# haoosz/FFR-Net

Hardware: AMD Instinct MI355X
Metric: face embeddings/sec (IR-SE50 + RecNet forward, 112x112 fp32) at batch 256 per GPU (higher is better)
Workload: dtype f32; 1 GPU; configs[2]: IR-SE50 + RecBlock (spatial+channel) forward, batch 256 per GPU, 112x112x3 fp32 -> f_new,f [512]; + all-gather of embeddings and pair cosine scores (112x96 of the BASELINE label cannot be embedded by the reference: BASELINE.md); batch_per_gpu=256, global_batch=256, parallelism=image-sharded x1, RCCL all-gather of embeddings

## Files before the change

ffr-net_amd/csrc/conv.cpp:

```cpp
#include "engine_internal.h"

namespace ffr_eng {

#ifdef FFR_TRACE
static int trace_igemm(ffr_handle* h, IgemmArgs& a, int tile, int nblocks, long long units, hipStream_t st) {
    unsigned long long* dbuf = nullptr;
    HIPCK(h, hipMalloc((void**)&dbuf, (size_t)nblocks * 8 * sizeof(unsigned long long)));
    a.trace = dbuf;
    HIPCK(h, launch_igemm(a, tile, nblocks, st));
    HIPCK(h, hipStreamSynchronize(st));
    std::vector<unsigned long long> t((size_t)nblocks * 8);
    HIPCK(h, hipMemcpy(t.data(), dbuf, t.size() * 8, hipMemcpyDeviceToHost));
    HIPCK(h, hipFree(dbuf));
    a.trace = nullptr;
    double acc[4] = {0, 0, 0, 0}, segs = 0, e1 = 0, e2 = 0, ghz = 0;
    unsigned long long r0 = ~0ull, r1 = 0, smax = 0;
    for (int b = 0; b < nblocks; ++b) {
        const unsigned long long* q = &t[(size_t)b * 8];
        for (int k = 0; k < 4; ++k) acc[k] += (double)q[k];
        segs += (double)q[4];
        ghz += (double)(q[0] + q[1] + q[2] + q[3]) / ((double)(q[6] - q[5]) * 10.0);
        e1 += (double)(q[7] >> 32); e2 += (double)(q[7] & 0xffffffffull);
        if (q[5] < r0) r0 = q[5];
        if (q[5] > smax) smax = q[5];
        if (q[6] > r1) r1 = q[6];
    }
    fprintf(stderr, "[igemm trace] tile %d blocks %d units %lld nkt %d segs/blk %.2f | per segment: setup %.0f prologue %.0f "
                    "loop %.0f (%.0f per K-tile) epilogue %.0f (first barrier at %.0f, C in LDS at %.0f) cyc | span %.1f us, starts within %.1f us, shader clock %.2f GHz\n",
            tile, nblocks, units, a.nkt, segs / nblocks, acc[0] / segs, acc[1] / segs, acc[2] / segs,
            acc[2] / ((double)units), acc[3] / segs, e1 / segs, e2 / segs, (double)(r1 - r0) / 100.0, (double)(smax - r0) / 100.0, ghz / nblocks);
    return FFR_OK;
}

static int trace_wino_mixed(ffr_handle* h, WinoMixedArgs& f, const ConvW& L, const ConvCall& c, hipStream_t st) {
    const int nbm = wino_mixed_blocks_launched(c.N, c.H, c.W, L.cout_pad, f.xcd_pairs);
    unsigned long long* dbuf = nullptr;
    HIPCK(h, hipMalloc((void**)&dbuf, (size_t)nbm * 12 * sizeof(unsigned long long)));
    HIPCK(h, hipMemsetAsync(dbuf, 0, (size_t)nbm * 12 * sizeof(unsigned long long), st));
    f.trace = dbuf;
    hipEvent_t e0, e1;
    HIPCK(h, hipEventCreate(&e0)); HIPCK(h, hipEventCreate(&e1));
    HIPCK(h, hipEventRecord(e0, st));
    HIPCK(h, launch_wino_fused_mixed(f, st));
    HIPCK(h, hipEventRecord(e1, st));
    HIPCK(h, hipStreamSynchronize(st));
    float ev_ms = 0.f;
    HIPCK(h, hipEventElapsedTime(&ev_ms, e0, e1));
    hipEventDestroy(e0); hipEventDestroy(e1);
    std::vector<unsigned long long> tr((size_t)nbm * 12);
    HIPCK(h, hipMemcpy(tr.data(), dbuf, tr.size() * 8, hipMemcpyDeviceToHost));
    HIPCK(h, hipFree(dbuf));
    double pro[4] = {0, 0, 0, 0}, loop[4] = {0, 0, 0, 0}, ep1[4] = {0, 0, 0, 0}, ep2[4] = {0, 0, 0, 0}, clk[4] = {0, 0, 0, 0};
    int cnt[4] = {0, 0, 0, 0};
// ... 240 lines not shown
        c2.x = c.x + px * c.in_pitch;
        c2.out = c.out + px * c.out_pitch;
        if (c.resid) c2.resid = c.resid + px * c.res_pitch;
        if (c.tile_sums) c2.tile_sums = c.tile_sums + (size_t)p.n_main * ((c.H + 3) / 4) * ((c.W + 3) / 4) * L.cout_pad;
        if (p.side) {
            HIPCK(h, hipEventRecord(h->ev_fork, st));
            HIPCK(h, hipStreamWaitEvent(p.side, h->ev_fork, 0));
            RC(run_conv(h, L, c2, p.side));
            HIPCK(h, hipEventRecord(h->ev_join, p.side));
            RC(run_conv(h, L, c1, st));
            HIPCK(h, hipStreamWaitEvent(st, h->ev_join, 0));
            return FFR_OK;
        }
        RC(run_conv(h, L, c1, st));
        return run_conv(h, L, c2, st);
    }
    IgemmArgs a{};
    a.x = c.x; a.w = L.w; a.bias = L.bias; a.slope = L.slope; a.resid = c.resid; a.out = c.out; a.zero = h->zero;
    a.N = c.N; a.H = c.H; a.W = c.W; a.Ho = Ho; a.Wo = Wo;
    a.in_pitch = c.in_pitch; a.cin_pad = L.cin_pad; a.R = L.R; a.S = L.S; a.stride = L.stride; a.pad = L.pad; a.pad_mode = L.pad_mode;
    a.M = (int)M; a.KK = L.R * L.S * L.cin_pad; a.nkt = a.KK / 32; a.nbatch = 1;
    a.cout_pad = L.cout_pad; a.cout_store = c.cout_store; a.out_pitch = c.out_pitch; a.out_coff = c.out_coff;
    a.res_pitch = c.res_pitch; a.border_bias = L.border; a.flags = c.flags;
    if (L.w3 && h->opt.igemm_split) { a.w3 = L.w3; a.w3_pstride = (long long)L.cout_pad * a.KK; }
    return run_gemm(h, a, c, flops, bytes, st);
}

int gemm_rows(ffr_handle* h, const Work& w, const float* A, int a_pitch, int K_pad, const float* W, const float* bias,
              int N_pad, float* out, int out_pitch, long long rows, const float* resid, int res_pitch, int flags,
              hipStream_t st) {
    ConvW cw;
    cw.cin = K_pad; cw.cin_pad = K_pad; cw.cout = N_pad; cw.cout_pad = N_pad; cw.R = 1; cw.S = 1; cw.stride = 1; cw.pad = 0;
    cw.pad_mode = 0; cw.border = 0; cw.w = const_cast<float*>(W); cw.bias = bias ? const_cast<float*>(bias) : h->zero;
    cw.slope = nullptr; cw.wu = nullptr;
    ConvCall c = conv_call(w, ConvForce::Direct);
    c.x = A; c.N = 1; c.H = 1; c.W = (int)rows; c.in_pitch = a_pitch; c.resid = resid; c.res_pitch = res_pitch;
    c.out = out; c.out_pitch = out_pitch; c.out_coff = 0; c.cout_store = N_pad; c.flags = flags;
    return run_conv(h, cw, c, st);
}

int gemm_batched(ffr_handle* h, const Work& w, const float* A, long long a_bstride, int K_pad, const float* W,
                 long long w_bstride, int N_pad, float* out, int out_pitch, long long out_bstride, int M, int nbatch,
                 hipStream_t st) {
    const double fl = 2.0 * nbatch * (double)M * N_pad * K_pad;
    return igemm_batched(h, conv_call(w, ConvForce::Direct), A, a_bstride, K_pad, W, w_bstride, N_pad, out, out_pitch, out_bstride, M,
                         nbatch, fl, 4.0 * nbatch * ((double)M * K_pad + (double)N_pad * K_pad + (double)M * N_pad), fl, st);
}
// ... 3 lines not shown
```

ffr-net_amd/csrc/engine.cpp:

```cpp
#include "engine_internal.h"

using namespace ffr;
using namespace ffr_eng;

namespace ffr_eng {

std::string g_err = "";

int fail(ffr_handle* h, int code, const char* fmt, ...) {
    char buf[512];
    va_list ap;
    va_start(ap, fmt);
    vsnprintf(buf, sizeof buf, fmt, ap);
    va_end(ap);
    if (h) h->err = buf; else g_err = buf;
    return code;
}

struct PlanLayer { ConvW* L; std::string name; int net; };

std::vector<PlanLayer> plan_layers(const ffr_handle* hc) {
    ffr_handle* h = const_cast<ffr_handle*>(hc);
    std::vector<PlanLayer> v;
    if (h->enc_loaded)
// ... 483 lines not shown
        RC(forward()); RC(compare(0));
        RC(read());
        if (err(0) <= half || p == 0) break;
    }
    if (achieved) for (int t = 0; t < 4; ++t) achieved[t] = have[t] ? rel(0, t) : -1.0;
    sv.keep = true;
    bool changed = false;
    for (auto& pr : sv.plan) changed |= pr.first->direct != pr.second;
    if (changed) plan_changed(h);
    else h->mixed_ready_n = 0;
    return FFR_OK;
}

namespace {
struct OptEntry { const char* name; int ffr_eng::Options::*i; long long ffr_eng::Options::*l; long long lo, hi; };
const OptEntry OPTIONS[] = {
    {"wino", &Options::wino, nullptr, 0, 1}, {"wino_mincin", &Options::wino_mincin, nullptr, 0, 1 << 20},
    {"wino_fused", &Options::wino_fused, nullptr, 0, 1},
    {"wf_phased_maxk", &Options::wf_phased_maxk, nullptr, 0, 1 << 20}, {"wf_minblocks", nullptr, &Options::wf_minblocks, 0, 1LL << 40},
    {"se_maxtiles", &Options::se_maxtiles, nullptr, 0, 1 << 20}, {"wf_tailsplit", &Options::wf_tailsplit, nullptr, 0, 1},
    {"gemm_stream", &Options::gemm_stream, nullptr, 0, 1}, {"sk_minunits", &Options::sk_minunits, nullptr, 1, 1 << 20},
    {"combine_v", &Options::combine_v, nullptr, 0, 1}, {"wf_mixed", &Options::wf_mixed, nullptr, 0, 1},
    {"channel_rows", &Options::channel_rows, nullptr, 0, 4}, {"igemm_split", &Options::igemm_split, nullptr, 0, 1},
    {"wf_trace", &Options::wf_trace, nullptr, 0, 1}, {"igemm_trace", &Options::igemm_trace, nullptr, 0, 1},
};
const OptEntry* find_option(const char* name) {
    if (name) for (const OptEntry& e : OPTIONS) if (!strcmp(e.name, name)) return &e;
    return nullptr;
}
}

int ffr_set_option(ffr_handle* h, const char* name, long long value) {
    if (!h) return fail(nullptr, FFR_ERR_ARG, "null handle");
    const OptEntry* e = find_option(name);
    if (!e) return fail(h, FFR_ERR_ARG, "ffr_set_option: unknown option '%s'", name ? name : "(null)");
    if (value < e->lo || value > e->hi) return fail(h, FFR_ERR_ARG, "ffr_set_option: %s = %lld is outside [%lld, %lld]", name, value, e->lo, e->hi);
    if (e->i == &Options::channel_rows && value == 3) return fail(h, FFR_ERR_ARG, "ffr_set_option: channel_rows is 0 (auto), 1, 2 or 4");
#ifndef FFR_TRACE
    if ((e->i == &Options::wf_trace || e->i == &Options::igemm_trace) && value)
        return fail(h, FFR_ERR_UNSUPPORTED, "ffr_set_option: %s needs a -DFFR_TRACE build of the library (tools/trace_build.py)", name);
#endif
    const long long old = e->i ? (long long)(h->opt.*(e->i)) : h->opt.*(e->l);
    if (old != value) ++h->generation;
    if (e->i) h->opt.*(e->i) = (int)value; else h->opt.*(e->l) = value;
    return FFR_OK;
}
// ... 154 lines not shown
```

ffr-net_amd/csrc/engine_internal.h:

```cpp
#pragma once
#include <hip/hip_runtime.h>

#include <algorithm>
#include <chrono>
#include <cmath>
#include <cstdarg>
#include <cstdio>
#include <cstdlib>
#include <cstring>
#include <initializer_list>
#include <map>
#include <string>
#include <vector>

#include "../../include/ffrnet.h"
#include "../../include/ffrnet_train.h"
#include "ffr_kernels.h"

namespace ffr_eng {

using namespace ffr;

struct TrainState;

// ... 12 lines not shown
};

struct Block {
    int cin = 0, depth = 0, stride = 1;
    bool has_sc = false;
    ConvW c1, c2, sc;
    float* fc1 = nullptr;
    float* fc2 = nullptr;
};

struct Options {
    int wino = 1;
    int wino_mincin = 64;
    int wino_fused = 1;
    int wf_phased_maxk = 128;
    long long wf_minblocks = 200;
    int se_maxtiles = 256;
    int wf_tailsplit = 1;
    int gemm_stream = 1;
    int sk_minunits = 18;
    int wf_mixed = 1;
    int channel_rows = 0;
    int igemm_split = 1;
    int combine_v = 1;
    int wf_trace = 0, igemm_trace = 0;
};

struct ProfRec {
    hipEvent_t e0, e1;
    int kc;
    double flops, bytes, fexec, fuse;
    bool side;
};

}

struct ffr_handle {
    int device = 0;
    int num_cus = 256;
    hipStream_t side = nullptr;
    hipEvent_t ev_fork = nullptr, ev_join = nullptr;
    std::string err;
    float* zero = nullptr;
    std::vector<void*> enc_allocs, rec_allocs;
    bool enc_loaded = false, rec_loaded = false;
    size_t enc_weight_bytes = 0, rec_weight_bytes = 0;
// ... 197 lines not shown
```

ffr-net_amd/csrc/ffr_kernels.h:

```cpp
#pragma once
#include <hip/hip_runtime.h>
#include <stdint.h>

#ifdef FFR_TRACE
#define FFR_TRACE_ON(p) ((p) != nullptr)
#else
#define FFR_TRACE_ON(p) false
#endif

namespace ffr {

struct IgemmArgs {
    const float* x;
    const float* w;
    const float* bias;
    const float* slope;
    const float* resid;
    float* out;
    const float* zero;
    float* partial;
    int* tickets;
    unsigned long long* trace;
    int N, H, W, Ho, Wo, in_pitch, cin_pad, R, S, stride, pad, pad_mode;
    int M, KK, nkt, granule;
    int nbatch;
    long long x_bstride, w_bstride, out_bstride;
    int cout_pad, cout_store, out_pitch, out_coff, res_pitch;
    int border_bias, flags;
    int mtiles, ntiles;
    const unsigned short* w3;
    long long w3_pstride;
};
enum { IGEMM_TILE_128x128 = 1, IGEMM_TILE_128x64 = 2, IGEMM_TILE_64x64 = 3, IGEMM_TILE_256x64 = 4,
       IGEMM_NTILES = 4 };
void igemm_tile_shape(int tile, int* bm, int* bn);
hipError_t igemm_init();
int igemm_resident_blocks(int tile, bool split = false);
hipError_t launch_split_weights(const float* w, unsigned short* planes, size_t n, hipStream_t stream);
hipError_t launch_igemm(const IgemmArgs& a, int tile, int nblocks, hipStream_t stream);

struct GemmStreamArgs {
    const float* A; const float* W; float* C;
    int M, K, Npad, nbatch;
    int mtiles, ntiles;
};
hipError_t gemm_stream_init();
hipError_t launch_gemm_stream(GemmStreamArgs a, int tile, int nblocks, hipStream_t stream);

hipError_t launch_wino_in(const float* x, float* V, int N, int H, int W, int pitch, int cin_pad, int pad_mode,
                          hipStream_t stream);
hipError_t launch_wino_weights(const float* W, float* U, int out_pad, int in_pad, hipStream_t stream, int chunked = 0);
hipError_t launch_wino_dout(const float* dy, float* dM, int N, int H, int W, int Cp, hipStream_t stream);
hipError_t launch_wino_dweights(const float* dU, float* grad, int out_pad, int in_pad, int accumulate, hipStream_t stream);
bool wino_out_in_supported(int H, int W, int C);
// ... 136 lines not shown
```

ffr-net_amd/csrc/igemm.hip:

```cpp
#include "ffr_kernels.h"

#include <utility>

namespace ffr {

typedef float f32x16 __attribute__((ext_vector_type(16)));
typedef float f32x4 __attribute__((ext_vector_type(4)));
typedef unsigned u32x4 __attribute__((ext_vector_type(4)));
typedef __bf16 bf16x8 __attribute__((ext_vector_type(8)));

#define LDS_PTR(p) ((__attribute__((address_space(3))) void*)(p))
#define GLB_PTR(p) ((const __attribute__((address_space(1))) void*)(p))

__device__ __forceinline__ unsigned cvt_pk_bf16(float lo, float hi) {
    unsigned r;
    asm("v_cvt_pk_bf16_f32 %0, %1, %2" : "=v"(r) : "v"(lo), "v"(hi));
    return r;
}

template <int BM, int BN, int WARPS_M, int WARPS_N, int PAD_MODE, bool SPLIT = false>
__global__ __launch_bounds__(256) void k_igemm(const IgemmArgs a) {
    constexpr int WM = BM / WARPS_M, WN = BN / WARPS_N;
    constexpr int TM = WM / 32, TN = WN / 32;
    constexpr int A_PT = BM / 32;
    constexpr int B_PT = SPLIT ? 3 * (BN / 64) : BN / 32;
    constexpr int STAGE_FLOATS = SPLIT ? BM * 32 + BN * 48 : (BM + BN) * 32;
    static_assert(WARPS_M * WARPS_N == 4, "4 waves");
    extern __shared__ __attribute__((aligned(16))) float smem[];
    constexpr int MAIN_FLOATS = (2 * STAGE_FLOATS > BM * (BN + 4)) ? 2 * STAGE_FLOATS : BM * (BN + 4);
    int* s_cls = reinterpret_cast<int*>(smem + MAIN_FLOATS);
    float* s_bias = smem + MAIN_FLOATS + BM + 4;

    const int wave = __builtin_amdgcn_readfirstlane(threadIdx.x >> 6);
    const int wm = wave / WARPS_N, wn = wave % WARPS_N;
    const int HoWo = a.Ho * a.Wo;

    const long long U = (long long)a.nbatch * a.mtiles * a.ntiles * a.nkt;
    const long long G = U / a.granule;
    long long u = (long long)blockIdx.x * G / gridDim.x * a.granule;
    const long long uend = (long long)(blockIdx.x + 1) * G / gridDim.x * a.granule;
    unsigned long long tr_acc[6] = {0, 0, 0, 0, 0, 0}, tr_seg = 0, tr_t = 0, tr_rt0 = 0;
    if (FFR_TRACE_ON(a.trace)) tr_rt0 = __builtin_amdgcn_s_memrealtime();
    while (u < uend) {
    const int tile_id = (int)(u / a.nkt);
    const int kb = (int)(u - (long long)tile_id * a.nkt);
    const int nk = (uend - u < (long long)(a.nkt - kb)) ? (int)(uend - u) : a.nkt - kb;
    u += nk;
    const int tpb = a.mtiles * a.ntiles;
    const int batch = tile_id / tpb;
    const int tile_b = tile_id - batch * tpb;
    const int nt = tile_b % a.ntiles, mt = tile_b / a.ntiles;
    const float* const xb = a.x + (long long)batch * a.x_bstride;
    const float* const wb = a.w + (long long)batch * a.w_bstride;
    float* const ob = a.out + (long long)batch * a.out_bstride;
    const int m0 = mt * BM, n0 = nt * BN;
    __syncthreads();
    __builtin_amdgcn_s_setprio(2);
    int tid = threadIdx.x;
    asm volatile("" : "+v"(tid));
    if (FFR_TRACE_ON(a.trace)) { tr_t = __builtin_amdgcn_s_memtime(); ++tr_seg; }
    const int lane = tid & 63;

    const int srow = tid >> 3;
    const int lch = (tid & 7) ^ ((srow >> 1) & 7);
    int a_pix[A_PT], a_h0[A_PT], a_w0[A_PT];
#pragma unroll
    for (int i = 0; i < A_PT; ++i) {
        int m = m0 + srow + 32 * i;
        if (m >= a.M) m = 0;
        if (a.H == 1 && a.N == 1) {
            a_pix[i] = 0;
            a_h0[i] = -a.pad;
            a_w0[i] = m * a.stride - a.pad;
        } else {
            const int n = m / HoWo;
            const int rem = m - n * HoWo;
            const int ho = rem / a.Wo;
            const int wo = rem - ho * a.Wo;
            a_pix[i] = n * a.H * a.W;
            a_h0[i] = ho * a.stride - a.pad;
            a_w0[i] = wo * a.stride - a.pad;
        }
    }
// ... 106 lines not shown
        for (int st = 0; st < 2; ++st) {
            pcA[st][0] = ((4 * st + 2 * fh) ^ fswz) * 4;
            pcA[st][1] = ((4 * st + 2 * fh + 1) ^ fswz) * 4;
            pcB[st] = ((2 * st + fh) ^ bswz) * 4;
        }
        const int fragB3 = BM * 32 + (wn * WN + frow) * 16;
        auto read_piece = [&](int slot, const float* stage, int st, int r) __attribute__((always_inline)) {
            if (r < 2 * TM) araw[r / 2][r % 2] = *reinterpret_cast<const f32x4*>(stage + fragA + (r / 2) * 32 * 32 + pcA[st][r % 2]);
            else {
                const int j = (r - 2 * TM) / 3, p = (r - 2 * TM) % 3;
                pb[slot][j][p] = *reinterpret_cast<const f32x4*>(stage + fragB3 + p * BN * 16 + j * 32 * 16 + pcB[st]);
            }
        };
        auto split_unit = [&](int slot, int u) __attribute__((always_inline)) {
            const int i = u / 8, e2 = (u / 2) % 4, v = e2 / 2, e = 2 * (e2 % 2);
            float lo = araw[i][v][e], hi = araw[i][v][e + 1];
            const unsigned w = cvt_pk_bf16(lo, hi);
            pa[slot][i][u % 2][e2] = w;
            lo -= __builtin_bit_cast(float, w << 16);
            hi -= __builtin_bit_cast(float, w & 0xffff0000u);
            if (u % 2) pa[slot][i][2][e2] = cvt_pk_bf16(lo, hi);
            else { araw[i][v][e] = lo; araw[i][v][e + 1] = hi; }
        };
        auto filler = [&]<int ST, bool LAST, int FI>(int cur, bool more) __attribute__((always_inline)) {
            constexpr int NDS = (ST == 1 && !LAST) ? ND : 0;
            if constexpr (FI < NR) read_piece(ST ^ 1, smem + (ST == 0 ? cur : cur ^ 1) * STAGE_FLOATS, ST ^ 1, FI);
            else if constexpr (FI < NR + NDS) { if (more) dma_piece(cur, FI - NR); }
            else split_unit(ST ^ 1, FI - NR - NDS);
        };
        auto gap = [&]<int ST, bool LAST, int G>(int cur, bool more) __attribute__((always_inline)) {
            constexpr int NDS = (ST == 1 && !LAST) ? ND : 0;
            constexpr int F = (ST == 0 || !LAST) ? NR + NDS + NU : 0;
            constexpr int q = G / (TM * TN), i = (G / TN) % TM, j = G % TN;
            acc[i][j] = __builtin_amdgcn_mfma_f32_32x32x16_bf16(__builtin_bit_cast(bf16x8, pa[ST][i][PA[q]]),
                                                               __builtin_bit_cast(bf16x8, pb[ST][j][PB[q]]), acc[i][j], 0, 0, 0);
            constexpr int F0 = (G * F + NQ - 1) / NQ, F1 = ((G + 1) * F + NQ - 1) / NQ;
            [&]<int... K>(std::integer_sequence<int, K...>) __attribute__((always_inline)) {
                (filler.template operator()<ST, LAST, F0 + K>(cur, more), ...);
            }(std::make_integer_sequence<int, F1 - F0>{});
            FFR_PIN;
        };
        auto step = [&]<int ST, bool LAST, int... G>(int cur, bool more, std::integer_sequence<int, G...>) __attribute__((always_inline)) {
            if (ST == 1 && !LAST) {
                asm volatile("s_waitcnt vmcnt(0)" ::: "memory");
                __syncthreads();
                FFR_PIN;
            }
            (gap.template operator()<ST, LAST, G>(cur, more), ...);
            if (ST == 1 && !LAST && more) { advance_tile(); FFR_PIN; }
        };
        auto tile_body = [&]<bool LAST>(int cur, bool more) __attribute__((always_inline)) {
            step.template operator()<0, LAST>(cur, more, std::make_integer_sequence<int, NQ>{});
            step.template operator()<1, LAST>(cur, more, std::make_integer_sequence<int, NQ>{});
        };
        if (FFR_TRACE_ON(a.trace)) { const unsigned long long t = __builtin_amdgcn_s_memtime(); tr_acc[0] += t - tr_t; tr_t = t; }
#pragma unroll
        for (int d = 0; d < ND; ++d) dma_piece(0, d);
        advance_tile();
        if (nk > 1) {
#pragma unroll
            for (int d = 0; d < ND; ++d) dma_piece(1, d);
            advance_tile();
            static_assert(ND < 16, "vmcnt immediate");
            __builtin_amdgcn_s_waitcnt(0x0F70 | ND);
        } else {
            asm volatile("s_waitcnt vmcnt(0)" ::: "memory");
        }
        asm volatile("s_waitcnt lgkmcnt(0)\n\ts_barrier" ::: "memory");
#pragma unroll
        for (int r = 0; r < NR; ++r) read_piece(0, smem, 0, r);
#pragma unroll
        for (int u = 0; u < NU; ++u) split_unit(0, u);
        FFR_PIN;
        if (FFR_TRACE_ON(a.trace)) { const unsigned long long t = __builtin_amdgcn_s_memtime(); tr_acc[1] += t - tr_t; tr_t = t; }
        __builtin_amdgcn_s_setprio(0);
#pragma unroll 1
        for (int it = 0; it + 1 < nk; ++it) tile_body.template operator()<false>(it & 1, it + 2 < nk);
        tile_body.template operator()<true>((nk - 1) & 1, false);
        __builtin_amdgcn_s_setprio(2);
        if (FFR_TRACE_ON(a.trace)) { const unsigned long long t = __builtin_amdgcn_s_memtime(); tr_acc[2] += t - tr_t; tr_t = t; }
    } else {
        constexpr int NQ = TM * TN * 4;
        constexpr int NR = TM + TN;
        constexpr int NDH = (ND + 1) / 2;
        static_assert(NR + NDH <= NQ, "fillers must fit the MFMA gaps of a chunk");
        f32x4 af[2][TM], bf[2][TN];

        auto read_piece = [&](int slot, const float* stage, int pcv, int r) {
            if (r < TM) af[slot][r] = *reinterpret_cast<const f32x4*>(stage + fragA + r * 32 * 32 + pcv);
            else bf[slot][r - TM] = *reinterpret_cast<const f32x4*>(stage + fragB + (r - TM) * 32 * 32 + pcv);
        };

        auto tile_body = [&]<bool LAST>(int cur) {
            const float* stage = smem + cur * STAGE_FLOATS;
            const float* stage_n = smem + (cur ^ 1) * STAGE_FLOATS;
#pragma unroll
            for (int q = 0; q < 4; ++q) {
                if (q == 3 && !LAST) {
                    asm volatile("s_waitcnt vmcnt(0)" ::: "memory");
                    __syncthreads();
                    FFR_PIN;
                }
#pragma unroll
                for (int g = 0; g < NQ; ++g) {
                    const int e = g / (TM * TN), i = (g / TN) % TM, j = g % TN;
                    acc[i][j] = __builtin_amdgcn_mfma_f32_32x32x2f32(af[q & 1][i][e], bf[q & 1][j][e], acc[i][j], 0, 0, 0);
                    if (g < NR) {
                        if (q < 3) read_piece((q + 1) & 1, stage, pc[q + 1], g);
                        else if (!LAST) read_piece(0, stage_n, pc[0], g);
                    } else if (!LAST && q < 2 && (g - NR) < NDH && q * NDH + (g - NR) < ND) {
                        dma_piece(cur ^ 1, q * NDH + (g - NR));
                    }
                    FFR_PIN;
                }
                if (q == 1 && !LAST) { advance_tile(); FFR_PIN; }
            }
        };

        if (FFR_TRACE_ON(a.trace)) { const unsigned long long t = __builtin_amdgcn_s_memtime(); tr_acc[0] += t - tr_t; tr_t = t; }
#pragma unroll
        for (int d = 0; d < ND; ++d) dma_piece(0, d);
        advance_tile();
        asm volatile("s_waitcnt vmcnt(0)" ::: "memory");
        __syncthreads();
#pragma unroll
        for (int r = 0; r < NR; ++r) read_piece(0, smem, pc[0], r);
        FFR_PIN;
        if (FFR_TRACE_ON(a.trace)) { const unsigned long long t = __builtin_amdgcn_s_memtime(); tr_acc[1] += t - tr_t; tr_t = t; }
        __builtin_amdgcn_s_setprio(0);
#pragma unroll 1
        for (int it = 0; it + 1 < nk; ++it) tile_body.template operator()<false>(it & 1);
        tile_body.template operator()<true>((nk - 1) & 1);
        __builtin_amdgcn_s_setprio(2);
        if (FFR_TRACE_ON(a.trace)) { const unsigned long long t = __builtin_amdgcn_s_memtime(); tr_acc[2] += t - tr_t; tr_t = t; }
    }
#undef FFR_PIN

    constexpr int LDC = BN + 4;
    constexpr int NQ4 = BN / 4;
    constexpr int RPP = 256 / NQ4;
    float* sC = smem;
    __syncthreads();
    if (FFR_TRACE_ON(a.trace)) { const unsigned long long t = __builtin_amdgcn_s_memtime(); tr_acc[4] += t - tr_t; }
#pragma unroll
    for (int i = 0; i < TM; ++i)
#pragma unroll
        for (int r = 0; r < 16; ++r) {
            const int ml = wm * WM + i * 32 + (r & 3) + 8 * (r >> 2) + 4 * fh;
#pragma unroll
            for (int j = 0; j < TN; ++j) sC[ml * LDC + wn * WN + j * 32 + frow] = acc[i][j][r];
        }
    __syncthreads();
    if (FFR_TRACE_ON(a.trace)) { const unsigned long long t = __builtin_amdgcn_s_memtime(); tr_acc[5] += t - tr_t; }
    const int erow = tid / NQ4, ecol = (tid - erow * NQ4) * 4;
    bool finish = true;
    if (nk != a.nkt) {
        const long long tb = (long long)tile_id * a.nkt;
        const int P = gridDim.x;
        const int b_lo = (int)(((tb + 1) * P - 1) / G), b_hi = (int)(((tb + a.nkt) * P - 1) / G);
        float* dst = a.partial + ((size_t)blockIdx.x * 2 + (kb != 0 ? 0 : 1)) * (BM * BN);
#pragma unroll 4
        for (int p = 0; p < BM / RPP; ++p) {
            const int ml = p * RPP + erow;
            const f32x4 val = *reinterpret_cast<const f32x4*>(sC + ml * LDC + ecol);
            asm volatile("global_store_dwordx4 %0, %1, off sc0 sc1\n\ts_nop 1" ::"v"(dst + ml * BN + ecol), "v"(val) : "memory");
        }
        asm volatile("s_waitcnt vmcnt(0)" ::: "memory");
        __syncthreads();
        if (tid == 0) {
            const int old = __hip_atomic_fetch_add(a.tickets + tile_id, 1, __ATOMIC_RELAXED, __HIP_MEMORY_SCOPE_AGENT);
            if (old == b_hi - b_lo) {
                __builtin_amdgcn_fence(__ATOMIC_ACQUIRE, "agent");
                asm volatile("s_waitcnt vmcnt(0)" ::: "memory");
                __hip_atomic_store(a.tickets + tile_id, 0, __ATOMIC_RELAXED, __HIP_MEMORY_SCOPE_AGENT);
            }
            s_cls[BM] = old;
        }
        __syncthreads();
        finish = s_cls[BM] == b_hi - b_lo;
// ... 5 lines not shown
                for (int bb = b_lo; bb <= b_hi; bb += 8) {
                    f32x4 v[8];
#pragma unroll
                    for (int k = 0; k < 8; ++k) {
                        const int bk = bb + k;
                        v[k] = (f32x4){0.f, 0.f, 0.f, 0.f};
                        if (bk <= b_hi) {
                            if (bk == (int)blockIdx.x) {
                                v[k] = *reinterpret_cast<const f32x4*>(sC + ml * LDC + ecol);
                            } else {
                                const int slot = ((long long)bk * G / P * a.granule > tb) ? 0 : 1;
                                v[k] = *reinterpret_cast<const f32x4*>(a.partial + ((size_t)bk * 2 + slot) * (BM * BN) + ml * BN + ecol);
                            }
                        }
                    }
#pragma unroll
                    for (int k = 0; k < 8; ++k)
                        if (bb + k <= b_hi) sum += v[k];
                }
                *reinterpret_cast<f32x4*>(sC + ml * LDC + ecol) = sum;
            }
        }
    }
    if (finish) {
        const int n = n0 + ecol;
        const bool vec = ((a.out_pitch | a.out_coff | a.res_pitch) & 3) == 0 && n + 4 <= a.cout_store && !(a.flags & 1);
        f32x4 slope4 = {1.f, 1.f, 1.f, 1.f};
        if (a.slope) slope4 = *reinterpret_cast<const f32x4*>(a.slope + n);
        const f32x4 bias0 = *reinterpret_cast<const f32x4*>(a.bias + n);
        constexpr int NP = BM / RPP;
        constexpr int BATCH = NP < 4 ? NP : 4;
        auto finish_tile = [&]<bool BORDER, bool RESID>() {
            f32x4 rs[BATCH], rn[BATCH];
            const int mrow = m0 + erow;
            float* optr = ob + (size_t)mrow * a.out_pitch + a.out_coff + n;
            const size_t ostep = (size_t)RPP * a.out_pitch;
            const float* rptr = RESID ? a.resid + (size_t)mrow * a.res_pitch + n : nullptr;
            const size_t rstep = (size_t)RPP * a.res_pitch;
            auto load_resid = [&](f32x4* dstv, int p0) {
#pragma unroll
                for (int k = 0; k < BATCH; ++k) {
                    dstv[k] = (f32x4){0.f, 0.f, 0.f, 0.f};
                    if (mrow + (p0 + k) * RPP < a.M) dstv[k] = *reinterpret_cast<const f32x4*>(rptr + (size_t)(p0 + k) * rstep);
                }
            };
            if (RESID) load_resid(rs, 0);
#pragma unroll
            for (int p0 = 0; p0 < NP; p0 += BATCH) {
                if (RESID && p0 + BATCH < NP) load_resid(rn, p0 + BATCH);
#pragma unroll
                for (int k = 0; k < BATCH; ++k) {
                    const int ml = (p0 + k) * RPP + erow;
                    f32x4 v = *reinterpret_cast<const f32x4*>(sC + ml * LDC + ecol);
                    if (BORDER) v += *reinterpret_cast<const f32x4*>(s_bias + s_cls[ml] * BN + ecol);
                    else v += bias0;
#pragma unroll
                    for (int e = 0; e < 4; ++e) v[e] = v[e] >= 0.f ? v[e] : v[e] * slope4[e];
                    if (RESID) v += rs[k];
                    if (m0 + ml < a.M) *reinterpret_cast<f32x4*>(optr) = v;
                    optr += ostep;
                }
                if (RESID) {
#pragma unroll
                    for (int k = 0; k < BATCH; ++k) rs[k] = rn[k];
                }
            }
        };
        if (vec) {
            if (a.border_bias) {
                if (a.resid) finish_tile.template operator()<true, true>();
                else finish_tile.template operator()<true, false>();
            } else {
                if (a.resid) finish_tile.template operator()<false, true>();
                else finish_tile.template operator()<false, false>();
            }
        } else {
#pragma unroll 1
            for (int p = 0; p < NP; ++p) {
                const int ml = p * RPP + erow;
                const int m = m0 + ml;
                if (m >= a.M) continue;
                f32x4 v = *reinterpret_cast<const f32x4*>(sC + ml * LDC + ecol);
                v += a.border_bias ? *reinterpret_cast<const f32x4*>(s_bias + s_cls[ml] * BN + ecol) : bias0;
#pragma unroll
                for (int e = 0; e < 4; ++e) {
                    if (n + e < a.cout_store) {
                        float x = v[e] >= 0.f ? v[e] : v[e] * slope4[e];
                        if (a.resid) x += a.resid[(size_t)m * a.res_pitch + n + e];
                        if (a.flags & 1) x = 1.0f / (1.0f + __expf(-x));
                        ob[(size_t)m * a.out_pitch + a.out_coff + n + e] = x;
                    }
                }
            }
        }
    }
    if (FFR_TRACE_ON(a.trace)) { const unsigned long long t = __builtin_amdgcn_s_memtime(); tr_acc[3] += t - tr_t; tr_t = t; }
    }
    if (FFR_TRACE_ON(a.trace) && threadIdx.x == 0) {
        unsigned long long* t = a.trace + (size_t)blockIdx.x * 8;
        t[0] = tr_acc[0]; t[1] = tr_acc[1]; t[2] = tr_acc[2]; t[3] = tr_acc[3]; t[4] = tr_seg;
        t[5] = tr_rt0; t[6] = __builtin_amdgcn_s_memrealtime(); t[7] = (tr_acc[4] << 32) | (tr_acc[5] & 0xffffffffull);
    }
}

void igemm_tile_shape(int tile, int* bm, int* bn) {
    switch (tile) {
        case IGEMM_TILE_128x128: *bm = 128; *bn = 128; break;
        case IGEMM_TILE_128x64: *bm = 128; *bn = 64; break;
        case IGEMM_TILE_64x64: *bm = 64; *bn = 64; break;
        case IGEMM_TILE_256x64: *bm = 256; *bn = 64; break;
        default: *bm = 0; *bn = 0;
    }
}

static size_t igemm_lds_bytes(int bm, int bn, bool split) {
    size_t stages = split ? (size_t)2 * (bm * 32 + bn * 48) : (size_t)2 * (bm + bn) * 32, ctile = (size_t)bm * (bn + 4);
    return (stages > ctile ? stages : ctile) * 4 + (size_t)(bm + 4) * 4 + (size_t)9 * bn * 4;
}

hipError_t igemm_init() {
    hipError_t e;
#define FFR_SET_LDS(BM, BN, WMM, WNN, SPLIT)                                                                   \
    e = hipFuncSetAttribute((const void*)k_igemm<BM, BN, WMM, WNN, 0, SPLIT>,                                  \
                            hipFuncAttributeMaxDynamicSharedMemorySize, (int)igemm_lds_bytes(BM, BN, SPLIT));  \
    if (e != hipSuccess) return e;                                                                             \
    e = hipFuncSetAttribute((const void*)k_igemm<BM, BN, WMM, WNN, 1, SPLIT>,                                  \
                            hipFuncAttributeMaxDynamicSharedMemorySize, (int)igemm_lds_bytes(BM, BN, SPLIT));  \
    if (e != hipSuccess) return e;
    FFR_SET_LDS(128, 128, 2, 2, false)
    FFR_SET_LDS(128, 64, 2, 2, false)
    FFR_SET_LDS(64, 64, 2, 2, false)
    FFR_SET_LDS(256, 64, 4, 1, false)
    FFR_SET_LDS(128, 128, 4, 1, true)
    FFR_SET_LDS(128, 64, 4, 1, true)
    FFR_SET_LDS(64, 64, 2, 2, true)
    FFR_SET_LDS(256, 64, 4, 1, true)
#undef FFR_SET_LDS
    return e;
}

int igemm_resident_blocks(int tile, bool split) {
    if (split) {
        switch (tile) {
            case IGEMM_TILE_128x128: return 1;
            case IGEMM_TILE_128x64: return 2;
            case IGEMM_TILE_64x64: return 3;
            case IGEMM_TILE_256x64: return 1;
            default: return 0;
        }
    }
    switch (tile) {
        case IGEMM_TILE_128x128: return 2;
        case IGEMM_TILE_128x64: return 3;
        case IGEMM_TILE_64x64: return 4;
        case IGEMM_TILE_256x64: return 1;
        default: return 0;
    }
}

hipError_t launch_igemm(const IgemmArgs& a, int tile, int nblocks, hipStream_t stream) {
    int bm, bn;
    igemm_tile_shape(tile, &bm, &bn);
    if (!bm || nblocks <= 0) return hipErrorInvalidValue;
    const bool split = a.w3 != nullptr;
    if (split && a.nbatch != 1) return hipErrorInvalidValue;
    dim3 grid((unsigned)nblocks, 1, 1);
    const size_t lds = igemm_lds_bytes(bm, bn, split);
#define FFR_LAUNCH(BM, BN, WMM, WNN, SPLIT)                                                                          \
    if (a.pad_mode == 1) hipLaunchKernelGGL((k_igemm<BM, BN, WMM, WNN, 1, SPLIT>), grid, dim3(256), lds, stream, a); \
    else hipLaunchKernelGGL((k_igemm<BM, BN, WMM, WNN, 0, SPLIT>), grid, dim3(256), lds, stream, a);
    if (split) {
        switch (tile) {
            case IGEMM_TILE_128x128: FFR_LAUNCH(128, 128, 4, 1, true) break;
            case IGEMM_TILE_128x64: FFR_LAUNCH(128, 64, 4, 1, true) break;
            case IGEMM_TILE_64x64: FFR_LAUNCH(64, 64, 2, 2, true) break;
            case IGEMM_TILE_256x64: FFR_LAUNCH(256, 64, 4, 1, true) break;
        }
    } else {
        switch (tile) {
            case IGEMM_TILE_128x128: FFR_LAUNCH(128, 128, 2, 2, false) break;
            case IGEMM_TILE_128x64: FFR_LAUNCH(128, 64, 2, 2, false) break;
            case IGEMM_TILE_64x64: FFR_LAUNCH(64, 64, 2, 2, false) break;
            case IGEMM_TILE_256x64: FFR_LAUNCH(256, 64, 4, 1, false) break;
        }
    }
#undef FFR_LAUNCH
    return hipGetLastError();
}

__global__ void k_split_weights(const float* __restrict__ w, unsigned short* __restrict__ planes, size_t n) {
// ... 19 lines not shown
```

Measured before the change: 17460 embeddings/s.

## Overlap igemm epilogue stores with next tile's main loop in split 128x128 kernel

For the split 128x128 implicit-GEMM tile, the C tile gets its own LDS region and double-buffered bias/class tables. This lets a full tile's bias+PReLU+store epilogue be deferred and drained piecewise inside the next segment's MFMA loop, instead of stalling the whole block. It also replaces __syncthreads with lgkmcnt-only barriers and a partial vmcnt wait so the pending stores are not waited on. The cost is a much larger LDS footprint (near the CU limit), which holds the kernel to one resident block, plus extra complexity and trace bookkeeping per cut/whole segment.

Measured after the change: 17460 embeddings/s (median of 2 runs). No clear change (+0.0%).

```diff
diff --git a/ffr-net_amd/csrc/conv.cpp b/ffr-net_amd/csrc/conv.cpp
--- a/ffr-net_amd/csrc/conv.cpp
+++ b/ffr-net_amd/csrc/conv.cpp
@@ -5,30 +5,40 @@
 #ifdef FFR_TRACE
 static int trace_igemm(ffr_handle* h, IgemmArgs& a, int tile, int nblocks, long long units, hipStream_t st) {
     unsigned long long* dbuf = nullptr;
-    HIPCK(h, hipMalloc((void**)&dbuf, (size_t)nblocks * 8 * sizeof(unsigned long long)));
+    HIPCK(h, hipMalloc((void**)&dbuf, (size_t)nblocks * 16 * sizeof(unsigned long long)));
     a.trace = dbuf;
     HIPCK(h, launch_igemm(a, tile, nblocks, st));
     HIPCK(h, hipStreamSynchronize(st));
-    std::vector<unsigned long long> t((size_t)nblocks * 8);
+    std::vector<unsigned long long> t((size_t)nblocks * 16);
     HIPCK(h, hipMemcpy(t.data(), dbuf, t.size() * 8, hipMemcpyDeviceToHost));
     HIPCK(h, hipFree(dbuf));
     a.trace = nullptr;
-    double acc[4] = {0, 0, 0, 0}, segs = 0, e1 = 0, e2 = 0, ghz = 0;
+    double acc[2][4] = {{0, 0, 0, 0}, {0, 0, 0, 0}}, segs[2] = {0, 0}, e1 = 0, e2 = 0, ghz = 0;
     unsigned long long r0 = ~0ull, r1 = 0, smax = 0;
     for (int b = 0; b < nblocks; ++b) {
-        const unsigned long long* q = &t[(size_t)b * 8];
-        for (int k = 0; k < 4; ++k) acc[k] += (double)q[k];
-        segs += (double)q[4];
-        ghz += (double)(q[0] + q[1] + q[2] + q[3]) / ((double)(q[6] - q[5]) * 10.0);
+        const unsigned long long* q = &t[(size_t)b * 16];
+        double cyc = 0;
+        for (int c = 0; c < 2; ++c) {
+            for (int k = 0; k < 4; ++k) { acc[c][k] += (double)q[8 * c + k]; cyc += (double)q[8 * c + k]; }
+            segs[c] += (double)q[8 * c + 4];
+        }
+        ghz += cyc / ((double)(q[6] - q[5]) * 10.0);
         e1 += (double)(q[7] >> 32); e2 += (double)(q[7] & 0xffffffffull);
         if (q[5] < r0) r0 = q[5];
         if (q[5] > smax) smax = q[5];
         if (q[6] > r1) r1 = q[6];
     }
-    fprintf(stderr, "[igemm trace] tile %d blocks %d units %lld nkt %d segs/blk %.2f | per segment: setup %.0f prologue %.0f "
+    const double sall = segs[0] + segs[1];
+    fprintf(stderr, "[igemm trace] tile %d%s%s blocks %d units %lld nkt %d segs/blk %.2f | per segment: setup %.0f prologue %.0f "
                     "loop %.0f (%.0f per K-tile) epilogue %.0f (first barrier at %.0f, C in LDS at %.0f) cyc | span %.1f us, starts within %.1f us, shader clock %.2f GHz\n",
-            tile, nblocks, units, a.nkt, segs / nblocks, acc[0] / segs, acc[1] / segs, acc[2] / segs,
-            acc[2] / ((double)units), acc[3] / segs, e1 / segs, e2 / segs, (double)(r1 - r0) / 100.0, (double)(smax - r0) / 100.0, ghz / nblocks);
+            tile, a.w3 ? " split" : "", a.w3 && a.overlap ? " overlap" : "", nblocks, units, a.nkt, sall / nblocks, (acc[0][0] + acc[1][0]) / sall,
+            (acc[0][1] + acc[1][1]) / sall, (acc[0][2] + acc[1][2]) / sall, (acc[0][2] + acc[1][2]) / ((double)units), (acc[0][3] + acc[1][3]) / sall,
+            e1 / sall, e2 / sall, (double)(r1 - r0) / 100.0, (double)(smax - r0) / 100.0, ghz / nblocks);
+    static const char* kind[2] = {"whole", "cut  "};
+    for (int c = 0; c < 2; ++c)
+        if (segs[c] > 0)
+            fprintf(stderr, "[igemm trace]   %s segments %.2f per block: setup %.0f prologue %.0f loop %.0f epilogue %.0f cyc\n", kind[c], segs[c] / nblocks,
+                    acc[c][0] / segs[c], acc[c][1] / segs[c], acc[c][2] / segs[c], acc[c][3] / segs[c]);
     return FFR_OK;
 }
 
@@ -315,7 +325,7 @@
     a.M = (int)M; a.KK = L.R * L.S * L.cin_pad; a.nkt = a.KK / 32; a.nbatch = 1;
     a.cout_pad = L.cout_pad; a.cout_store = c.cout_store; a.out_pitch = c.out_pitch; a.out_coff = c.out_coff;
     a.res_pitch = c.res_pitch; a.border_bias = L.border; a.flags = c.flags;
-    if (L.w3 && h->opt.igemm_split) { a.w3 = L.w3; a.w3_pstride = (long long)L.cout_pad * a.KK; }
+    if (L.w3 && h->opt.igemm_split) { a.w3 = L.w3; a.w3_pstride = (long long)L.cout_pad * a.KK; a.overlap = h->opt.igemm_overlap; }
     return run_gemm(h, a, c, flops, bytes, st);
 }
 
diff --git a/ffr-net_amd/csrc/engine.cpp b/ffr-net_amd/csrc/engine.cpp
--- a/ffr-net_amd/csrc/engine.cpp
+++ b/ffr-net_amd/csrc/engine.cpp
@@ -529,6 +529,7 @@
     {"gemm_stream", &Options::gemm_stream, nullptr, 0, 1}, {"sk_minunits", &Options::sk_minunits, nullptr, 1, 1 << 20},
     {"combine_v", &Options::combine_v, nullptr, 0, 1}, {"wf_mixed", &Options::wf_mixed, nullptr, 0, 1},
     {"channel_rows", &Options::channel_rows, nullptr, 0, 4}, {"igemm_split", &Options::igemm_split, nullptr, 0, 1},
+    {"igemm_overlap", &Options::igemm_overlap, nullptr, 0, 1},
     {"wf_trace", &Options::wf_trace, nullptr, 0, 1}, {"igemm_trace", &Options::igemm_trace, nullptr, 0, 1},
 };
 const OptEntry* find_option(const char* name) {
diff --git a/ffr-net_amd/csrc/engine_internal.h b/ffr-net_amd/csrc/engine_internal.h
--- a/ffr-net_amd/csrc/engine_internal.h
+++ b/ffr-net_amd/csrc/engine_internal.h
@@ -58,6 +58,7 @@
     int wf_mixed = 1;
     int channel_rows = 0;
     int igemm_split = 1;
+    int igemm_overlap = 1;
     int combine_v = 1;
     int wf_trace = 0, igemm_trace = 0;
 };
diff --git a/ffr-net_amd/csrc/ffr_kernels.h b/ffr-net_amd/csrc/ffr_kernels.h
--- a/ffr-net_amd/csrc/ffr_kernels.h
+++ b/ffr-net_amd/csrc/ffr_kernels.h
@@ -30,6 +30,7 @@
     int mtiles, ntiles;
     const unsigned short* w3;
     long long w3_pstride;
+    int overlap;
 };
 enum { IGEMM_TILE_128x128 = 1, IGEMM_TILE_128x64 = 2, IGEMM_TILE_64x64 = 3, IGEMM_TILE_256x64 = 4,
        IGEMM_NTILES = 4 };
diff --git a/ffr-net_amd/csrc/igemm.hip b/ffr-net_amd/csrc/igemm.hip
--- a/ffr-net_amd/csrc/igemm.hip
+++ b/ffr-net_amd/csrc/igemm.hip
@@ -27,9 +27,14 @@
     constexpr int STAGE_FLOATS = SPLIT ? BM * 32 + BN * 48 : (BM + BN) * 32;
     static_assert(WARPS_M * WARPS_N == 4, "4 waves");
     extern __shared__ __attribute__((aligned(16))) float smem[];
-    constexpr int MAIN_FLOATS = (2 * STAGE_FLOATS > BM * (BN + 4)) ? 2 * STAGE_FLOATS : BM * (BN + 4);
-    int* s_cls = reinterpret_cast<int*>(smem + MAIN_FLOATS);
-    float* s_bias = smem + MAIN_FLOATS + BM + 4;
+    constexpr int RING_FLOATS = 2 * STAGE_FLOATS, CT_FLOATS = BM * (BN + 4);
+    constexpr int MAIN_FLOATS = (RING_FLOATS > CT_FLOATS) ? RING_FLOATS : CT_FLOATS;
+    constexpr int TBL_FLOATS = BM + 4 + 9 * BN;
+    constexpr bool OVL = SPLIT && BM == 128 && BN == 128;
+    static_assert(!OVL || (RING_FLOATS + CT_FLOATS + 2 * TBL_FLOATS) * 4 <= 160 * 1024, "overlap layout exceeds the LDS of a CU");
+    const bool ovl = OVL && a.overlap;
+    float* const sC = ovl ? smem + RING_FLOATS : smem;
+    float* const tbl0 = smem + (ovl ? RING_FLOATS + CT_FLOATS : MAIN_FLOATS);
 
     const int wave = __builtin_amdgcn_readfirstlane(threadIdx.x >> 6);
     const int wm = wave / WARPS_N, wn = wave % WARPS_N;
@@ -39,8 +44,40 @@
     const long long G = U / a.granule;
     long long u = (long long)blockIdx.x * G / gridDim.x * a.granule;
     const long long uend = (long long)(blockIdx.x + 1) * G / gridDim.x * a.granule;
-    unsigned long long tr_acc[6] = {0, 0, 0, 0, 0, 0}, tr_seg = 0, tr_t = 0, tr_rt0 = 0;
+    unsigned long long tr_acc[2][6] = {{0, 0, 0, 0, 0, 0}, {0, 0, 0, 0, 0, 0}}, tr_seg[2] = {0, 0}, tr_t = 0, tr_rt0 = 0;
     if (FFR_TRACE_ON(a.trace)) tr_rt0 = __builtin_amdgcn_s_memrealtime();
+
+    constexpr int LDC = BN + 4;
+    constexpr int NQ4 = BN / 4;
+    constexpr int RPP = 256 / NQ4;
+    constexpr int NP = BM / RPP;
+    int pd_left = 0, pd_par = 0;
+    float* pd_optr = nullptr;
+    f32x4 pd_slope = {1.f, 1.f, 1.f, 1.f}, dr_v[2], dr_b[2];
+    const size_t pd_ostep = (size_t)RPP * a.out_pitch;
+    auto drain_read = [&](int k) __attribute__((always_inline)) {
+        const int t = threadIdx.x, ml = (NP - pd_left + k) * RPP + (t >> 5);
+        const float* tb = tbl0 + pd_par * TBL_FLOATS;
+        dr_v[k] = *reinterpret_cast<const f32x4*>(sC + ml * LDC + (t & 31) * 4);
+        const int cls = reinterpret_cast<const int*>(tb)[ml];
+        dr_b[k] = *reinterpret_cast<const f32x4*>(tb + BM + 4 + cls * BN + (t & 31) * 4);
+    };
+    auto drain_store = [&](int k) __attribute__((always_inline)) {
+        f32x4 v = dr_v[k] + dr_b[k];
+#pragma unroll
+        for (int e = 0; e < 4; ++e) v[e] = v[e] >= 0.f ? v[e] : v[e] * pd_slope[e];
+        asm volatile("global_store_dwordx4 %0, %1, off\n\ts_nop 1" ::"v"(pd_optr), "v"(v) : "memory");
+        pd_optr += pd_ostep;
+    };
+    auto flush_pending = [&]() __attribute__((always_inline)) {
+#pragma unroll 1
+        while (pd_left > 0) {
+            drain_read(0); drain_read(1);
+            drain_store(0); drain_store(1);
+            pd_left -= 2;
+        }
+    };
+    int seg = 0;
     while (u < uend) {
     const int tile_id = (int)(u / a.nkt);
     const int kb = (int)(u - (long long)tile_id * a.nkt);
@@ -54,11 +91,16 @@
     const float* const wb = a.w + (long long)batch * a.w_bstride;
     float* const ob = a.out + (long long)batch * a.out_bstride;
     const int m0 = mt * BM, n0 = nt * BN;
-    __syncthreads();
+    const bool cutseg = nk != a.nkt;
+    const int par = ovl ? (seg & 1) : 0;
+    ++seg;
+    int* s_cls = reinterpret_cast<int*>(tbl0 + par * TBL_FLOATS);
+    float* s_bias = tbl0 + par * TBL_FLOATS + BM + 4;
+    if (!ovl) __syncthreads();
     __builtin_amdgcn_s_setprio(2);
     int tid = threadIdx.x;
     asm volatile("" : "+v"(tid));
-    if (FFR_TRACE_ON(a.trace)) { tr_t = __builtin_amdgcn_s_memtime(); ++tr_seg; }
+    if (FFR_TRACE_ON(a.trace)) { tr_t = __builtin_amdgcn_s_memtime(); ++tr_seg[cutseg]; }
     const int lane = tid & 63;
 
     const int srow = tid >> 3;
@@ -211,38 +253,50 @@
             if (u % 2) pa[slot][i][2][e2] = cvt_pk_bf16(lo, hi);
             else { araw[i][v][e] = lo; araw[i][v][e + 1] = hi; }
         };
-        auto filler = [&]<int ST, bool LAST, int FI>(int cur, bool more) __attribute__((always_inline)) {
+        auto filler = [&]<int ST, bool LAST, bool DRAIN, int FI>(int cur, bool more) __attribute__((always_inline)) {
             constexpr int NDS = (ST == 1 && !LAST) ? ND : 0;
+            constexpr int NDR = (ST == 1 && DRAIN) ? 4 : 0;
             if constexpr (FI < NR) read_piece(ST ^ 1, smem + (ST == 0 ? cur : cur ^ 1) * STAGE_FLOATS, ST ^ 1, FI);
             else if constexpr (FI < NR + NDS) { if (more) dma_piece(cur, FI - NR); }
-            else split_unit(ST ^ 1, FI - NR - NDS);
-        };
-        auto gap = [&]<int ST, bool LAST, int G>(int cur, bool more) __attribute__((always_inline)) {
+            else if constexpr (FI < NR + NDS + NDR) {
+                constexpr int D = FI - NR - NDS;
+                if constexpr (D < 2) drain_read(D);
+                else drain_store(D - 2);
+            } else split_unit(ST ^ 1, FI - NR - NDS - NDR);
+        };
+        auto gap = [&]<int ST, bool LAST, bool DRAIN, int G>(int cur, bool more) __attribute__((always_inline)) {
             constexpr int NDS = (ST == 1 && !LAST) ? ND : 0;
-            constexpr int F = (ST == 0 || !LAST) ? NR + NDS + NU : 0;
+            constexpr int F = (ST == 0 || !LAST) ? NR + NDS + NU + ((ST == 1 && DRAIN) ? 4 : 0) : 0;
             constexpr int q = G / (TM * TN), i = (G / TN) % TM, j = G % TN;
             acc[i][j] = __builtin_amdgcn_mfma_f32_32x32x16_bf16(__builtin_bit_cast(bf16x8, pa[ST][i][PA[q]]),
                                                                __builtin_bit_cast(bf16x8, pb[ST][j][PB[q]]), acc[i][j], 0, 0, 0);
             constexpr int F0 = (G * F + NQ - 1) / NQ, F1 = ((G + 1) * F + NQ - 1) / NQ;
             [&]<int... K>(std::integer_sequence<int, K...>) __attribute__((always_inline)) {
-                (filler.template operator()<ST, LAST, F0 + K>(cur, more), ...);
+                (filler.template operator()<ST, LAST, DRAIN, F0 + K>(cur, more), ...);
             }(std::make_integer_sequence<int, F1 - F0>{});
             FFR_PIN;
         };
-        auto step = [&]<int ST, bool LAST, int... G>(int cur, bool more, std::integer_sequence<int, G...>) __attribute__((always_inline)) {
+        auto step = [&]<int ST, bool LAST, bool DRAIN, int... G>(int cur, bool more, bool prevd, std::integer_sequence<int, G...>) __attribute__((always_inline)) {
             if (ST == 1 && !LAST) {
-                asm volatile("s_waitcnt vmcnt(0)" ::: "memory");
-                __syncthreads();
+                if constexpr (OVL) {
+                    if (prevd) asm volatile("s_waitcnt vmcnt(2)" ::: "memory");
+                    else asm volatile("s_waitcnt vmcnt(0)" ::: "memory");
+                    asm volatile("s_waitcnt lgkmcnt(0)\n\ts_barrier" ::: "memory");
+                } else {
+                    asm volatile("s_waitcnt vmcnt(0)" ::: "memory");
+                    __syncthreads();
+                }
                 FFR_PIN;
             }
-            (gap.template operator()<ST, LAST, G>(cur, more), ...);
+            (gap.template operator()<ST, LAST, DRAIN, G>(cur, more), ...);
+            if (ST == 1 && DRAIN) pd_left -= 2;
             if (ST == 1 && !LAST && more) { advance_tile(); FFR_PIN; }
         };
-        auto tile_body = [&]<bool LAST>(int cur, bool more) __attribute__((always_inline)) {
-            step.template operator()<0, LAST>(cur, more, std::make_integer_sequence<int, NQ>{});
-            step.template operator()<1, LAST>(cur, more, std::make_integer_sequence<int, NQ>{});
-        };
-        if (FFR_TRACE_ON(a.trace)) { const unsigned long long t = __builtin_amdgcn_s_memtime(); tr_acc[0] += t - tr_t; tr_t = t; }
+        auto tile_body = [&]<bool LAST, bool DRAIN>(int cur, bool more, bool prevd) __attribute__((always_inline)) {
+            step.template operator()<0, LAST, DRAIN>(cur, more, prevd, std::make_integer_sequence<int, NQ>{});
+            step.template operator()<1, LAST, DRAIN>(cur, more, prevd, std::make_integer_sequence<int, NQ>{});
+        };
+        if (FFR_TRACE_ON(a.trace)) { const unsigned long long t = __builtin_amdgcn_s_memtime(); tr_acc[cutseg][0] += t - tr_t; tr_t = t; }
 #pragma unroll
         for (int d = 0; d < ND; ++d) dma_piece(0, d);
         advance_tile();
@@ -261,13 +315,22 @@
 #pragma unroll
         for (int u = 0; u < NU; ++u) split_unit(0, u);
         FFR_PIN;
-        if (FFR_TRACE_ON(a.trace)) { const unsigned long long t = __builtin_amdgcn_s_memtime(); tr_acc[1] += t - tr_t; tr_t = t; }
+        if (FFR_TRACE_ON(a.trace)) { const unsigned long long t = __builtin_amdgcn_s_memtime(); tr_acc[cutseg][1] += t - tr_t; tr_t = t; }
         __builtin_amdgcn_s_setprio(0);
+        if constexpr (OVL) {
+            int it = 0;
 #pragma unroll 1
-        for (int it = 0; it + 1 < nk; ++it) tile_body.template operator()<false>(it & 1, it + 2 < nk);
-        tile_body.template operator()<true>((nk - 1) & 1, false);
+            for (; it + 1 < nk && pd_left > 0; ++it) tile_body.template operator()<false, true>(it & 1, it + 2 < nk, it > 0);
+            const int it0 = it;
+#pragma unroll 1
+            for (; it + 1 < nk; ++it) tile_body.template operator()<false, false>(it & 1, it + 2 < nk, it == it0 && it0 > 0);
+        } else {
+#pragma unroll 1
+            for (int it = 0; it + 1 < nk; ++it) tile_body.template operator()<false, false>(it & 1, it + 2 < nk, false);
+        }
+        tile_body.template operator()<true, false>((nk - 1) & 1, false, false);
         __builtin_amdgcn_s_setprio(2);
-        if (FFR_TRACE_ON(a.trace)) { const unsigned long long t = __builtin_amdgcn_s_memtime(); tr_acc[2] += t - tr_t; tr_t = t; }
+        if (FFR_TRACE_ON(a.trace)) { const unsigned long long t = __builtin_amdgcn_s_memtime(); tr_acc[cutseg][2] += t - tr_t; tr_t = t; }
     } else {
         constexpr int NQ = TM * TN * 4;
         constexpr int NR = TM + TN;
@@ -306,7 +369,7 @@
             }
         };
 
-        if (FFR_TRACE_ON(a.trace)) { const unsigned long long t = __builtin_amdgcn_s_memtime(); tr_acc[0] += t - tr_t; tr_t = t; }
+        if (FFR_TRACE_ON(a.trace)) { const unsigned long long t = __builtin_amdgcn_s_memtime(); tr_acc[cutseg][0] += t - tr_t; tr_t = t; }
 #pragma unroll
         for (int d = 0; d < ND; ++d) dma_piece(0, d);
         advance_tile();
@@ -315,22 +378,23 @@
 #pragma unroll
         for (int r = 0; r < NR; ++r) read_piece(0, smem, pc[0], r);
         FFR_PIN;
-        if (FFR_TRACE_ON(a.trace)) { const unsigned long long t = __builtin_amdgcn_s_memtime(); tr_acc[1] += t - tr_t; tr_t = t; }
+        if (FFR_TRACE_ON(a.trace)) { const unsigned long long t = __builtin_amdgcn_s_memtime(); tr_acc[cutseg][1] += t - tr_t; tr_t = t; }
         __builtin_amdgcn_s_setprio(0);
 #pragma unroll 1
         for (int it = 0; it + 1 < nk; ++it) tile_body.template operator()<false>(it & 1);
         tile_body.template operator()<true>((nk - 1) & 1);
         __builtin_amdgcn_s_setprio(2);
-        if (FFR_TRACE_ON(a.trace)) { const unsigned long long t = __builtin_amdgcn_s_memtime(); tr_acc[2] += t - tr_t; tr_t = t; }
+        if (FFR_TRACE_ON(a.trace)) { const unsigned long long t = __builtin_amdgcn_s_memtime(); tr_acc[cutseg][2] += t - tr_t; tr_t = t; }
     }
 #undef FFR_PIN
 
-    constexpr int LDC = BN + 4;
-    constexpr int NQ4 = BN / 4;
-    constexpr int RPP = 256 / NQ4;
-    float* sC = smem;
-    __syncthreads();
-    if (FFR_TRACE_ON(a.trace)) { const unsigned long long t = __builtin_amdgcn_s_memtime(); tr_acc[4] += t - tr_t; }
+    if constexpr (OVL) flush_pending();
+    auto lds_barrier = [&]() __attribute__((always_inline)) {
+        if constexpr (OVL) asm volatile("s_waitcnt lgkmcnt(0)\n\ts_barrier" ::: "memory");
+        else __syncthreads();
+    };
+    lds_barrier();
+    if (FFR_TRACE_ON(a.trace)) { const unsigned long long t = __builtin_amdgcn_s_memtime(); tr_acc[cutseg][4] += t - tr_t; }
 #pragma unroll
     for (int i = 0; i < TM; ++i)
 #pragma unroll
@@ -339,11 +403,11 @@
 #pragma unroll
             for (int j = 0; j < TN; ++j) sC[ml * LDC + wn * WN + j * 32 + frow] = acc[i][j][r];
         }
-    __syncthreads();
-    if (FFR_TRACE_ON(a.trace)) { const unsigned long long t = __builtin_amdgcn_s_memtime(); tr_acc[5] += t - tr_t; }
+    lds_barrier();
+    if (FFR_TRACE_ON(a.trace)) { const unsigned long long t = __builtin_amdgcn_s_memtime(); tr_acc[cutseg][5] += t - tr_t; }
     const int erow = tid / NQ4, ecol = (tid - erow * NQ4) * 4;
     bool finish = true;
-    if (nk != a.nkt) {
+    if (cutseg) {
         const long long tb = (long long)tile_id * a.nkt;
         const int P = gridDim.x;
         const int b_lo = (int)(((tb + 1) * P - 1) / G), b_hi = (int)(((tb + a.nkt) * P - 1) / G);
@@ -395,13 +459,15 @@
             }
         }
     }
+    const bool defer = OVL && ovl && !cutseg && !a.resid && m0 + BM <= a.M && n0 + BN <= a.cout_store &&
+                       ((a.out_pitch | a.out_coff) & 3) == 0 && !(a.flags & 1);
+    if (defer) { pd_left = NP; pd_par = par; }
     if (finish) {
         const int n = n0 + ecol;
         const bool vec = ((a.out_pitch | a.out_coff | a.res_pitch) & 3) == 0 && n + 4 <= a.cout_store && !(a.flags & 1);
         f32x4 slope4 = {1.f, 1.f, 1.f, 1.f};
         if (a.slope) slope4 = *reinterpret_cast<const f32x4*>(a.slope + n);
         const f32x4 bias0 = *reinterpret_cast<const f32x4*>(a.bias + n);
-        constexpr int NP = BM / RPP;
         constexpr int BATCH = NP < 4 ? NP : 4;
         auto finish_tile = [&]<bool BORDER, bool RESID>() {
             f32x4 rs[BATCH], rn[BATCH];
@@ -439,7 +505,14 @@
                 }
             }
         };
-        if (vec) {
+        if (defer) {
+            pd_slope = slope4;
+            if (!a.border_bias) {
+                if (erow == 0) *reinterpret_cast<f32x4*>(s_bias + ecol) = bias0;
+                if (tid < BM) s_cls[tid] = 0;
+            }
+            pd_optr = ob + (size_t)(m0 + erow) * a.out_pitch + a.out_coff + n;
+        } else if (vec) {
             if (a.border_bias) {
                 if (a.resid) finish_tile.template operator()<true, true>();
                 else finish_tile.template operator()<true, false>();
@@ -467,12 +540,20 @@
             }
         }
     }
-    if (FFR_TRACE_ON(a.trace)) { const unsigned long long t = __builtin_amdgcn_s_memtime(); tr_acc[3] += t - tr_t; tr_t = t; }
+    if (FFR_TRACE_ON(a.trace)) { const unsigned long long t = __builtin_amdgcn_s_memtime(); tr_acc[cutseg][3] += t - tr_t; tr_t = t; }
+    }
+    if constexpr (OVL) {
+        if (FFR_TRACE_ON(a.trace)) tr_t = __builtin_amdgcn_s_memtime();
+        flush_pending();
+        if (FFR_TRACE_ON(a.trace)) tr_acc[0][3] += __builtin_amdgcn_s_memtime() - tr_t;
     }
     if (FFR_TRACE_ON(a.trace) && threadIdx.x == 0) {
-        unsigned long long* t = a.trace + (size_t)blockIdx.x * 8;
-        t[0] = tr_acc[0]; t[1] = tr_acc[1]; t[2] = tr_acc[2]; t[3] = tr_acc[3]; t[4] = tr_seg;
-        t[5] = tr_rt0; t[6] = __builtin_amdgcn_s_memrealtime(); t[7] = (tr_acc[4] << 32) | (tr_acc[5] & 0xffffffffull);
+        unsigned long long* t = a.trace + (size_t)blockIdx.x * 16;
+        for (int c = 0; c < 2; ++c) {
+            t[8 * c + 0] = tr_acc[c][0]; t[8 * c + 1] = tr_acc[c][1]; t[8 * c + 2] = tr_acc[c][2]; t[8 * c + 3] = tr_acc[c][3]; t[8 * c + 4] = tr_seg[c];
+        }
+        t[5] = tr_rt0; t[6] = __builtin_amdgcn_s_memrealtime();
+        t[7] = ((tr_acc[0][4] + tr_acc[1][4]) << 32) | ((tr_acc[0][5] + tr_acc[1][5]) & 0xffffffffull);
     }
 }
 
@@ -486,19 +567,22 @@
     }
 }
 
-static size_t igemm_lds_bytes(int bm, int bn, bool split) {
+static constexpr size_t igemm_lds_bytes(int bm, int bn, bool split, bool overlap = false) {
     size_t stages = split ? (size_t)2 * (bm * 32 + bn * 48) : (size_t)2 * (bm + bn) * 32, ctile = (size_t)bm * (bn + 4);
-    return (stages > ctile ? stages : ctile) * 4 + (size_t)(bm + 4) * 4 + (size_t)9 * bn * 4;
-}
+    size_t tables = (size_t)(bm + 4) + (size_t)9 * bn;
+    if (overlap && split && bm == 128 && bn == 128) return (stages + ctile + 2 * tables) * 4;
+    return ((stages > ctile ? stages : ctile) + tables) * 4;
+}
+static_assert(igemm_lds_bytes(128, 128, true, true) == 159776 && igemm_lds_bytes(128, 128, true, true) <= 160 * 1024, "overlap layout: 80 KB ring + 66 KB C tile + 2 x 5 KB tables must fit the CU's 160 KB");
 
 hipError_t igemm_init() {
     hipError_t e;
-#define FFR_SET_LDS(BM, BN, WMM, WNN, SPLIT)                                                                   \
-    e = hipFuncSetAttribute((const void*)k_igemm<BM, BN, WMM, WNN, 0, SPLIT>,                                  \
-                            hipFuncAttributeMaxDynamicSharedMemorySize, (int)igemm_lds_bytes(BM, BN, SPLIT));  \
-    if (e != hipSuccess) return e;                                                                             \
-    e = hipFuncSetAttribute((const void*)k_igemm<BM, BN, WMM, WNN, 1, SPLIT>,                                  \
-                            hipFuncAttributeMaxDynamicSharedMemorySize, (int)igemm_lds_bytes(BM, BN, SPLIT));  \
+#define FFR_SET_LDS(BM, BN, WMM, WNN, SPLIT)                                                                         \
+    e = hipFuncSetAttribute((const void*)k_igemm<BM, BN, WMM, WNN, 0, SPLIT>,                                        \
+                            hipFuncAttributeMaxDynamicSharedMemorySize, (int)igemm_lds_bytes(BM, BN, SPLIT, true));  \
+    if (e != hipSuccess) return e;                                                                                   \
+    e = hipFuncSetAttribute((const void*)k_igemm<BM, BN, WMM, WNN, 1, SPLIT>,                                        \
+                            hipFuncAttributeMaxDynamicSharedMemorySize, (int)igemm_lds_bytes(BM, BN, SPLIT, true));  \
     if (e != hipSuccess) return e;
     FFR_SET_LDS(128, 128, 2, 2, false)
     FFR_SET_LDS(128, 64, 2, 2, false)
@@ -538,7 +622,7 @@
     const bool split = a.w3 != nullptr;
     if (split && a.nbatch != 1) return hipErrorInvalidValue;
     dim3 grid((unsigned)nblocks, 1, 1);
-    const size_t lds = igemm_lds_bytes(bm, bn, split);
+    const size_t lds = igemm_lds_bytes(bm, bn, split, a.overlap != 0);
 #define FFR_LAUNCH(BM, BN, WMM, WNN, SPLIT)                                                                          \
     if (a.pad_mode == 1) hipLaunchKernelGGL((k_igemm<BM, BN, WMM, WNN, 1, SPLIT>), grid, dim3(256), lds, stream, a); \
     else hipLaunchKernelGGL((k_igemm<BM, BN, WMM, WNN, 0, SPLIT>), grid, dim3(256), lds, stream, a);
```
